# suchapalaver/krust

Measured on AMD Instinct MI355X. Metric: canonical k-mers/s at k=21, 100M x 150bp reads; bit-exact vs krust CPU, higher is better.
Workload: dtype u64; 1 GPU; S100M: 100000000 x 150 bp reads per GPU (rank r: reads [r x 100000000, (r + 1) x 100000000)), k=21, genome 2^27 bp, seed 20260130; resident in HBM; k=21, reads_per_gpu=100000000, distinct_per_gpu=1085824844, table_slots=2147483648, capacity_hint=1115311478, parallelism=reads sharded x1

## Files before the change

krust_amd/csrc/batch.hip:

```cpp
#include "ctx.hip.h"
#include "level1_api.h"

namespace khi {

template <bool QUAL>
void launch_count(kh_ctx *c, const uint8_t *abase, const uint8_t *qbase, int qaligned, u64 vbeg, u64 vend,
                  u64 wlo, u64 tile0, u64 ntiles) {
    u64 blocks = ntiles < (u64)grid_cap() ? ntiles : (u64)grid_cap();
    uint32_t tpb = (uint32_t)((ntiles + blocks - 1) / blocks);
    blocks = (ntiles + tpb - 1) / tpb;
    uint32_t thr = 0;
    if (QUAL) {
        int t = c->minq + 33;
        thr = (uint32_t)(t > 255 ? 255 : t);
    }
    hipLaunchKernelGGL(kh::count_direct_kernel<QUAL>, dim3((unsigned)blocks), dim3(kh::BLOCK), 0, c->stream, abase,
                       qbase, qaligned, vbeg, vend, wlo, tile0, ntiles, tpb, c->k, thr, table_geom(c, c->table, c->cap), c->d_ctr);
}

struct RangeArgs {
    const uint8_t *abase, *qbase;
    int qaligned;
    bool use_qual;
    u64 vbeg, vend, wlo;
    double survive = 1.0;
};

constexpr int KH_RETRY_FULL_SIZE = 1000;
constexpr int KH_RETRY_WIDE = 1001;

u64 sized_for(u64 n, double survive) {
    if (survive >= 1.0) return n;
    const double e = (double)n * (survive * 1.125 + 1.0 / 64) + 65536.0;
    return e >= (double)n ? n : (u64)e;
}

uint32_t qual_thr(const kh_ctx *c) {
    int t = c->minq + 33;
    return (uint32_t)(t > 255 ? 255 : t);
}

template <typename PT>
void launch_region(kh_ctx *c, const kh::PartGeom &g, u64 nregions, u64 hot, const u64 *bend, bool narrow, u64 skip, u64 expect);
bool region_small_groups(const kh_ctx *c, u64 expect, u64 nregions) {
    const int forced = c->knobs.region_nt;
    if (forced) return forced == 512;
    const double keys = c->est_keys ? (double)(c->distinct_known + c->est_keys) : c->hinted ? (double)c->hint_keys : (double)(c->distinct_known + expect);
    return !(keys > 0.6 * (double)c->cap && expect / nregions > 16384);
}
static bool want_heads(const kh_ctx *c) { return c->comm != nullptr || c->exports_seen || c->knobs.heads_always; }
template <>
void launch_region<u64>(kh_ctx *c, const kh::PartGeom &g, u64 nregions, u64 hot, const u64 *bend, bool, u64 skip, u64 expect) {
    const kh::TableGeom tg = table_geom(c, c->table, c->cap);
#define KH_REGION64(FRESH, NT) \
// ... 168 lines not shown
                               (const uint8_t *)c->rfail, c->d_ctr);
            HIP_TRY(c, hipMemsetAsync(&c->d_ctr->part_failed, 0, sizeof(u64), c->stream));
        }
        HIP_TRY(c, hipGetLastError());
        rc = sync_counters(c);
        if (rc != KH_OK) return rc;
    }
    if (c->h_ctr->hot) {
        const u64 nhot = c->h_ctr->hot, hot_total = c->h_ctr->hot_total;
        const bool crowded = nhot > nregions / 64 && (double)(c->distinct_known + hot_total) > LOAD_HARD * (double)c->cap;
        const bool hot_narrow = sizeof(PT) == 4 && c->narrow && !crowded && c->h_ctr->kmers + hot_total < 0xFFFFFFFFull;
        if (c->trace)
            fprintf(stderr, "[kmerhip] %llu hot bucket(s) (more than %llu payloads each, %llu together) counted apart from the region pass%s\n", nhot,
                    hot_cut, hot_total, hot_narrow ? ", into the 8-byte image" : "");
        if (!hot_narrow && (rc = ensure_wide(c)) != KH_OK) return rc;
        if (crowded) {
            u64 newcap = c->cap * 2;
            while ((double)(c->distinct_known + hot_total) > LOAD_TARGET * (double)newcap) newcap *= 2;
            StageTimer t(c, ST_GROW);
            if ((rc = grow_to(c, newcap)) != KH_OK) return rc;
        }
        {
            StageTimer t(c, ST_MISC);
            if (hot_narrow)
                hipLaunchKernelGGL((kh::hot_buckets_kernel<PT, sizeof(PT) == 4>), dim3(kh::HOT_GRID), dim3(kh::BLOCK), 0, c->stream, table_geom(c, c->table, c->cap), g,
                                   (const PT *)bufB, (const u64 *)c->bstart, bend, (const uint32_t *)c->hot_list, nhot, c->d_ctr, c->ntab);
            else
                hipLaunchKernelGGL((kh::hot_buckets_kernel<PT, false>), dim3(kh::HOT_GRID), dim3(kh::BLOCK), 0, c->stream, table_geom(c, c->table, c->cap), g,
                                   (const PT *)bufB, (const u64 *)c->bstart, bend, (const uint32_t *)c->hot_list, nhot, c->d_ctr, (u64 *)nullptr);
            HIP_TRY(c, hipMemsetAsync(&c->d_ctr->hot, 0, 2 * sizeof(u64), c->stream));
        }
        HIP_TRY(c, hipGetLastError());
        c->rheads_valid = false;
        if ((rc = sync_counters(c)) != KH_OK) return rc;
    }
    if ((double)c->distinct_known > LOAD_PART * (double)c->cap) {
        u64 newcap = c->cap * 2;
        while ((double)c->distinct_known > LOAD_TARGET * (double)newcap) newcap *= 2;
        StageTimer t(c, ST_GROW);
        rc = grow_to(c, newcap);
        if (rc != KH_OK) return rc;
    }
    return KH_OK;
}

template <typename PT>
int partition_batch(kh_ctx *c, const RangeArgs &ra, GeomChoice &gc, u64 tile0, u64 ntiles, bool size_from_sample, double range_scale, bool sized_narrow, bool may_narrow) {
    constexpr bool CHUNKED = true;
    kh::PartGeom &g = gc.g;
    const u64 P1 = 1ull << g.p1_bits;
    const u64 n_all = ntiles * kh::PART_TILE;
    const bool estimated = ra.survive < 1.0;
    const u64 n_ub = sized_for(n_all, ra.survive);
    const u64 pool_chunks = (n_ub / kh::CHUNK_PAY) + (n_ub / kh::CHUNK_PAY) / 24 + (u64)PART_G1 * (P1 + kh::POOL_GRAB) + 1024;
    const u64 max_blocks = pool_chunks / kh::CPB + P1 + 1;
    int rc;
    if (!c->moff) {
        u64 z = 0;
        z = 0;
        if ((rc = ensure_buf(c, &c->moff, &z, (u64)kh::MAX_P1 + 1, "hipMalloc(moff)")) != KH_OK) return rc;
        z = 0;
        if ((rc = ensure_buf(c, &c->nch, &z, (u64)kh::MAX_P1 + 1, "hipMalloc(nch)")) != KH_OK) return rc;
        z = 0;
        if ((rc = ensure_buf(c, &c->info, &z, 8, "hipMalloc(info)")) != KH_OK) return rc;
        z = 0;
        if ((rc = ensure_buf(c, &c->pcount, &z, (u64)kh::MAX_P1, "hipMalloc(pcount)")) != KH_OK) return rc;
        z = 0;
        if ((rc = ensure_buf(c, &c->pstart, &z, (u64)kh::MAX_P1 + 1, "hipMalloc(pstart)")) != KH_OK) return rc;
        z = 0;
        if ((rc = ensure_buf(c, &c->pool_next, &z, 1, "hipMalloc(pool_next)")) != KH_OK) return rc;
        z = 0;
        if ((rc = ensure_buf(c, &c->ptotal, &z, (u64)kh::MAX_P1, "hipMalloc(ptotal)")) != KH_OK) return rc;
        z = 0;
        if ((rc = ensure_buf(c, &c->pcap, &z, (u64)kh::MAX_P1, "hipMalloc(pcap)")) != KH_OK) return rc;
        z = 0;
        if ((rc = ensure_buf(c, &c->ovf, &z, 4, "hipMalloc(ovf)")) != KH_OK) return rc;
        z = 0;
        if ((rc = ensure_buf(c, &c->heavy, &z, (u64)kh::MAX_P1, "hipMalloc(heavy)")) != KH_OK) return rc;
    }
    if ((rc = ensure_buf(c, &c->blocks, &c->blocks_cap, max_blocks, "hipMalloc(blocks)")) != KH_OK) return rc;
    if (c->pool_cap < pool_chunks) {
        u64 z = c->chunk_part ? c->pool_cap : 0;
        if ((rc = ensure_buf(c, &c->chunk_part, &z, pool_chunks, "hipMalloc(chunk_part)")) != KH_OK) return rc;
        z = c->fill8 ? c->pool_cap : 0;
        if ((rc = ensure_buf(c, &c->fill8, &z, pool_chunks, "hipMalloc(fill8)")) != KH_OK) return rc;
        z = c->plist ? c->pool_cap : 0;
        if ((rc = ensure_buf(c, &c->plist, &z, pool_chunks, "hipMalloc(plist)")) != KH_OK) return rc;
        c->pool_cap = pool_chunks;
    }
    const u64 a_bytes = pool_chunks * kh::CHUNK_PAY * sizeof(PT);
    if (c->key_cap < a_bytes) {
        u64 z = c->keysA ? c->key_cap : 0;
        if ((rc = ensure_buf(c, &c->keysA, &z, a_bytes, "hipMalloc(keysA)")) != KH_OK) return rc;
        c->key_cap = a_bytes;
    }
    const uint32_t est_np = size_from_sample ? (uint32_t)std::min<u64>(16, std::max<u64>(1, (2ull << 20) / std::max<u64>(1, n_ub / P1))) : 0u;
    constexpr uint32_t EST_P0 = 517;
    u64 est_slots = 0;
    uint32_t est_sub = 0;
    if (size_from_sample) {
        while (est_sub < 6 && (n_ub / P1) >> (est_sub + 1) >= (1ull << 19)) ++est_sub;
        est_slots = 1ull << 16;
        while (est_slots < 3 * (u64)est_np * ((n_ub / P1 >> est_sub) + 1)) est_slots *= 2;
        if ((rc = ensure_buf(c, &c->est_set, &c->est_set_cap, est_slots, "hipMalloc(distinct sample)")) != KH_OK) return rc;
    }

    const uint32_t tpb = (uint32_t)((ntiles + PART_G1 - 1) / PART_G1);
// ... 512 lines not shown
```

krust_amd/csrc/level1.hip.h:

```cpp
#pragma once
#include <utility>

#include "part_common.hip.h"
#include "window.hip.h"

namespace kh {

struct ChunkDst {
    u64 a;
    u64 b;
};
constexpr u64 CHUNK_DST_DROP = 1ull << 63;

template <bool QUAL, int MODE, bool FAST, typename PT, int KT>
__global__ __launch_bounds__(PART_NT) void part1_scatter_chunked_kernel(
    const uint8_t *__restrict__ abase, const uint8_t *__restrict__ qbase, int qaligned, u64 vbeg, u64 vend, u64 wlo,
    u64 tile0, u64 ntiles, uint32_t tiles_per_block, uint32_t k, uint32_t thr, PartGeom g, PT *__restrict__ pool,
    uint16_t *__restrict__ chunk_part, uint8_t *__restrict__ fill8, u64 *__restrict__ pool_next, u64 pool_chunks,
    Counters *ctr) {
    constexpr int ROUNDS = sizeof(PT) == 8 ? 2 : 1;
    constexpr int WPR = CHUNK / ROUNDS;
    constexpr int RTILE = PART_NT * WPR;
    __shared__ uint32_t s_code[2][PART_NT + 2];
    __shared__ uint16_t s_val[2][PART_NT + 2];
    __shared__ PT s_stage[RTILE + 2];
    __shared__ uint16_t s_pid[RTILE + 2];
    __shared__ uint32_t s_cnt[MAX_P1];
    __shared__ uint32_t s_meta[MAX_P1];
    __shared__ ChunkDst s_dst[MAX_P1];
    __shared__ uint32_t s_wsum[4];
    __shared__ uint16_t s_lofs[MAX_P1];
    __shared__ u64 s_priv_next, s_priv_end;
    const int tid = threadIdx.x;
    if (KT) k = KT;
    const uint32_t p1b = (KT == 21 && FAST) ? 10u : g.p1_bits;
    s_cnt[tid] = 0;
    if (tid == 0) {
        s_priv_next = atomicAdd(pool_next, (u64)POOL_GRAB);
        s_priv_end = s_priv_next + POOL_GRAB;
    }
    u64 cur = 0;
    uint32_t fill = CHUNK_PAY;
    bool have_chunk = false;
    const u64 tb = tile0 + (u64)blockIdx.x * tiles_per_block;
    u64 te = tb + tiles_per_block;
    if (te > tile0 + ntiles) te = tile0 + ntiles;
    int buf = 0;
    uint32_t lost = 0;
    __syncthreads();
    {
        const RawChunk raw0 = load_raw<QUAL>(abase, qbase, qaligned, chunk_pos<PART_NT>(tb, tid), vbeg, tb < te ? vend : 0);
        stage_encode<QUAL, PART_NT>(s_code, s_val, 0, true, tid, raw0, abase, qbase, qaligned, tb, vbeg, vend, thr);
    }
    for (u64 t = tb; t < te; ++t, buf ^= 1) {
        __syncthreads();
// ... 87 lines not shown
            __syncthreads();
            s_cnt[tid] = 0;
            if (tid == 0 && s_priv_next + POOL_LOW > s_priv_end) {
                s_priv_next = atomicAdd(pool_next, (u64)POOL_GRAB);
                s_priv_end = s_priv_next + POOL_GRAB;
            }
            if (h == 0)
                stage_encode<QUAL, PART_NT>(s_code, s_val, buf ^ 1, false, tid, raw, abase, qbase, qaligned, t + 1, vbeg, vend, thr);
#if !(KH_ABL & 4)
#pragma unroll 2
            for (uint32_t i = tid; i < total; i += PART_NT) {
                const uint32_t p = s_pid[i];
                const uint32_t meta = s_meta[p];
                const ChunkDst d = s_dst[p];
                const uint32_t e = i - (meta & 0xFFFFu);
#if KH_ABL & 2
                if (s_stage[i] == 0x12345678u && e == 77 && d.a == 5) pool[0] = 1;
#else
                if (e < (meta >> 16)) pool[d.a + i] = s_stage[i];
                else if (d.b != CHUNK_DST_DROP) pool[d.b + i] = s_stage[i];
#endif
            }
#endif
            if (h + 1 < ROUNDS) __syncthreads();
        }
    }
    if (have_chunk) fill8[cur] = (uint8_t)(fill - 1);
    const u64 l = wave_sum((u64)lost);
    if (lane_id() == 0 && l) atomicAdd(&ctr->failed, l);
}

constexpr uint32_t P1B_CAP = 32;
constexpr uint32_t P1B_WORDS = MAX_P1 * P1B_CAP;

__device__ __forceinline__ uint32_t rev2_complement(uint32_t x) {
    const uint32_t y = __builtin_bitreverse32(~x);
    return ((y >> 1) & 0x55555555u) | ((y & 0x55555555u) << 1);
}

typedef __attribute__((address_space(3))) uint32_t lds_u32;
#ifndef KH_L1_SWIZZLE
#define KH_L1_SWIZZLE 1
#endif
constexpr uint32_t L1_ROT_MASK = KH_L1_SWIZZLE ? 0x70u : 0u;
constexpr uint32_t K21_CNT_OFF = 0;
constexpr uint32_t K21_BIN_OFF = (MAX_P1 + PART_NT) * 4;
constexpr uint32_t K21_TRASH_OFF = K21_BIN_OFF + P1B_WORDS * 4;
constexpr uint32_t K21_WASTE0 = 0x10000u;
__device__ __forceinline__ uint32_t l1_bin_offset(uint32_t p) { return (p << 7) | ((p << 4) & L1_ROT_MASK); }
__device__ __forceinline__ uint32_t l1_word(uint32_t p, uint32_t w) { return w ^ (((p << 4) & L1_ROT_MASK) >> 2); }
__device__ __forceinline__ uint32_t l1_word64(uint32_t p, uint32_t w) { return w ^ (((p << 4) & L1_ROT_MASK) >> 3); }
__device__ __forceinline__ uint32_t l1_unit(uint32_t p, uint32_t u) { return u ^ (((p << 4) & L1_ROT_MASK) >> 4); }

template <bool QUAL, int MODE, bool FAST, int KW>
__global__ __launch_bounds__(PART_NT) void part1_bins_kernel(
    const uint8_t *__restrict__ abase, const uint8_t *__restrict__ qbase, int qaligned, u64 vbeg, u64 vend, u64 wlo,
    u64 tile0, u64 ntiles, uint32_t tiles_per_block, uint32_t k_rt, uint32_t thr, PartGeom g, uint32_t *__restrict__ pool,
    uint16_t *__restrict__ chunk_part, uint8_t *__restrict__ fill8, u64 *__restrict__ pool_next, u64 pool_chunks,
    Counters *ctr) {
    constexpr bool ASM = KW != 0;
    const uint32_t k = ASM ? (uint32_t)KW : k_rt, p1b = ASM ? 10u : g.p1_bits;
    constexpr int HALF = CHUNK / 2;
    constexpr uint32_t SEG = 16;
    __shared__ __attribute__((aligned(16))) uint32_t s_mem[(K21_TRASH_OFF + 16) / 4];
    __shared__ uint32_t s_code[2][PART_NT + 2];
    __shared__ uint16_t s_val[2][PART_NT + 2];
    __shared__ uint32_t s_flag;
    __shared__ u64 s_priv_next, s_priv_end;
    uint32_t *const s_cnt = s_mem + K21_CNT_OFF / 4;
    uint32_t *const s_bin = s_mem + K21_BIN_OFF / 4;
    __attribute__((address_space(3))) char *const lds = (__attribute__((address_space(3))) char *)s_mem;
    const int tid = threadIdx.x;
    s_cnt[tid] = 0;
    s_cnt[MAX_P1 + tid] = K21_WASTE0;
    if (tid == 0) {
        s_flag = 0;
        s_priv_next = atomicAdd(pool_next, (u64)POOL_GRAB);
        s_priv_end = s_priv_next + POOL_GRAB;
    }
    u64 cur = 0;
    uint32_t fill = CHUNK_PAY;
    uint32_t res = 0;
    bool have_chunk = false;
    const u64 tb = tile0 + (u64)blockIdx.x * tiles_per_block;
    u64 te = tb + tiles_per_block;
    if (te > tile0 + ntiles) te = tile0 + ntiles;
    int buf = 0;
    uint32_t lost = 0;
    const uint32_t waste = K21_CNT_OFF + 4u * (MAX_P1 + (uint32_t)tid);
    uint32_t *const bin = s_bin + (uint32_t)tid * P1B_CAP;
    __syncthreads();
    auto take_chunk = [&](u64 &first) -> bool {
        first = atomicAdd(&s_priv_next, 1ull);
        if (first + 1 > s_priv_end) first = atomicAdd(pool_next, 1ull);
        if (first + 1 > pool_chunks) return false;
        chunk_part[first] = (uint16_t)tid;
        return true;
    };
    auto flush = [&](uint32_t c) -> uint32_t {
        const uint32_t nseg = c / SEG;
        const uint32_t bseg = min(nseg, P1B_CAP / SEG);
        const uint32_t r = c % SEG;
        uint32_t nout = nseg;
        u64 dst[P1B_CAP / SEG];
        const uint32_t space = (CHUNK_PAY - fill) / SEG;
        u64 ib = 0;
        uint32_t ntaken = 0;
        u64 run_a = cur * CHUNK_PAY + fill, run_b = 0;
        if (nseg > space) {
            const uint32_t need = nseg - space;
            const uint32_t nnew = (need * SEG + CHUNK_PAY - 1) / CHUNK_PAY;
            u64 first = 0;
            bool ok = true;
            if (nnew == 1) ok = take_chunk(first);
            else {
                first = atomicAdd(pool_next, (u64)nnew);
                ok = first + nnew <= pool_chunks;
                if (ok) for (uint32_t q = 0; q < nnew; ++q) chunk_part[first + q] = (uint16_t)tid;
            }
            if (!ok) {
                lost += need * SEG;
                nout = space;
            } else {
                ib = first;
                ntaken = nnew;
                run_b = first * CHUNK_PAY - (u64)space * SEG;
                cur = first + nnew - 1;
                fill = need * SEG - (nnew - 1) * CHUNK_PAY;
                have_chunk = true;
            }
        } else {
            fill += nseg * SEG;
        }
        (void)ib; (void)ntaken;
#pragma unroll
        for (uint32_t sg = 0; sg < P1B_CAP / SEG; ++sg) dst[sg] = (sg < space ? run_a : run_b) + (u64)sg * SEG;
        const uint32_t nb = min(bseg, nout);
        uint4 *const bin4 = reinterpret_cast<uint4 *>(bin);
#pragma unroll
        for (uint32_t sg = 0; sg < P1B_CAP / SEG; ++sg)
            if (sg < nb) {
                uint4 *d = reinterpret_cast<uint4 *>(pool + dst[sg]);
                const uint4 x0 = bin4[l1_unit(tid, 4 * sg)], x1 = bin4[l1_unit(tid, 4 * sg + 1)], x2 = bin4[l1_unit(tid, 4 * sg + 2)],
                            x3 = bin4[l1_unit(tid, 4 * sg + 3)];
                d[0] = x0; d[1] = x1; d[2] = x2; d[3] = x3;
            }
        if (c <= P1B_CAP) {
            if (bseg) {
                const uint32_t nu = (r + 3u) / 4u;
                for (uint32_t i = 0; i < nu; ++i) bin4[l1_unit(tid, i)] = bin4[l1_unit(tid, 4 * bseg + i)];
            }
            s_cnt[tid] = r * 4u;
        } else {
            bin[l1_word(tid, 16)] = (uint32_t)run_a;
            bin[l1_word(tid, 17)] = (uint32_t)(run_a >> 32);
            bin[l1_word(tid, 18)] = (uint32_t)run_b;
            bin[l1_word(tid, 19)] = (uint32_t)(run_b >> 32);
            bin[l1_word(tid, 20)] = space * SEG;
            bin[l1_word(tid, 21)] = nout * SEG;
            bin[l1_word(tid, 22)] = nseg * SEG;
            s_cnt[tid] = (r - (c - P1B_CAP)) * 4u;
        }
        s_cnt[MAX_P1 + tid] = K21_WASTE0;
        return r;
    };
    {
        const RawChunk raw0 = load_raw<QUAL>(abase, qbase, qaligned, chunk_pos<PART_NT>(tb, tid), vbeg, tb < te ? vend : 0);
        stage_encode<QUAL, PART_NT>(s_code, s_val, 0, true, tid, raw0, abase, qbase, qaligned, tb, vbeg, vend, thr);
    }
    for (u64 t = tb; t < te; ++t, buf ^= 1) {
        __syncthreads();
        const RawChunk raw = load_raw<QUAL>(abase, qbase, qaligned, chunk_pos<PART_NT>(t + 1, tid), vbeg, t + 1 < te ? vend : 0);
        const WinCtx w = stage_collect<PART_NT>(s_code, s_val, buf, tid, t);
        const uint32_t good = window_good(w, k, wlo);
        const uint32_t w0 = (uint32_t)w.lo64, w1 = (uint32_t)(w.lo64 >> 32), w2 = w.hi;
        const uint32_t c0 = ASM ? rev2_complement(w2) : 0u, c1 = ASM ? rev2_complement(w1) : 0u, c2 = ASM ? rev2_complement(w0) : 0u;
        Roller roll;
        if (!ASM) roll.init(w, k, wlo);
        auto window = [&](int j, uint32_t &pay, uint32_t &cnta, uint32_t &binb) {
            u64 key;
            const bool ok = roll.next(j, key);
            uint32_t p1 = 0;
            pay = 0;
            if (!QUAL || ok) {
                if (FAST) {
                    hash_p1_pay32<MODE>(k, p1b, key, p1, pay);
                } else {
                    const u64 H = part_hash<MODE>(g, key);
                    pay = Pay<uint32_t>::make(key, H, g);
                    p1 = p1_of_hash(H, g);
                }
            }
            cnta = ok ? K21_CNT_OFF + 4u * p1 : waste;
            binb = l1_bin_offset(p1);
        };
#define KH_W21(J)                                                                                            \
    {                                                                                                        \
        uint32_t cnta;                                                                                       \
        if constexpr (ASM) {                                                                                 \
            uint32_t flo, fhi, rlo, rhi;                                                                     \
            win_fields<KW ? KW : 21, J>(w0, w1, w2, c0, c1, c2, flo, fhi, rlo, rhi);                         \
            win_hash32<KW ? KW : 21, J>(flo, fhi, rlo, rhi, good, waste, L1_ROT_MASK, pay[(J) % HALF], cnta, binb[(J) % HALF]); \
        } else window(J, pay[(J) % HALF], cnta, binb[(J) % HALF]);                                           \
        rk[(J) % HALF] = __hip_atomic_fetch_add((lds_u32 *)(lds + cnta), 4u, __ATOMIC_RELAXED, __HIP_MEMORY_SCOPE_WORKGROUP); \
    }
#pragma unroll
        for (int h = 0; h < 2; ++h) {
            uint32_t omask = 0;
            {
                uint32_t pay[HALF], binb[HALF], rk[HALF];
                if (h == 0) { KH_W21(0) KH_W21(1) KH_W21(2) KH_W21(3) KH_W21(4) KH_W21(5) KH_W21(6) KH_W21(7) }
                else { KH_W21(8) KH_W21(9) KH_W21(10) KH_W21(11) KH_W21(12) KH_W21(13) KH_W21(14) KH_W21(15) }
                uint32_t racc = 0;
#pragma unroll
                for (int j = 0; j < HALF; ++j) {
                    const uint32_t r4 = rk[j];
                    *(lds_u32 *)(lds + K21_BIN_OFF + (r4 < 4u * P1B_CAP ? (binb[j] ^ r4) : K21_TRASH_OFF - K21_BIN_OFF)) = pay[j];
                    racc |= r4;
                }
                if (racc & (K21_WASTE0 - 4u * P1B_CAP)) {
                    s_flag = 1u;
#pragma unroll
                    for (int j = 0; j < HALF; ++j)
                        if (rk[j] >= 4u * P1B_CAP && rk[j] < K21_WASTE0) omask |= 1u << j;
                }
            }
            if (h == 1 && tid == 0 && s_priv_next + 2 * POOL_LOW > s_priv_end) {
                s_priv_next = atomicAdd(pool_next, (u64)POOL_GRAB);
                s_priv_end = s_priv_next + POOL_GRAB;
            }
            __syncthreads();
            const bool slow = s_flag != 0u;
            if (h == 0)
                stage_encode<QUAL, PART_NT>(s_code, s_val, buf ^ 1, false, tid, raw, abase, qbase, qaligned, t + 1, vbeg, vend, thr);
            res = flush(s_cnt[tid] >> 2);
            if (slow) {
                __syncthreads();
                if (omask) {
                    Roller again;
                    again.init(w, k, wlo);
#pragma unroll
                    for (int j = 0; j < CHUNK; ++j) {
                        u64 key;
                        again.next(j, key);
                        if (j / HALF == h && ((omask >> (j % HALF)) & 1u)) {
                            uint32_t p, pv;
                            if (FAST) {
                                hash_p1_pay32<MODE>(k, p1b, key, p, pv);
                            } else {
                                const u64 H = part_hash<MODE>(g, key);
                                pv = Pay<uint32_t>::make(key, H, g);
                                p = p1_of_hash(H, g);
                            }
                            uint32_t *const pbin = s_bin + p * P1B_CAP;
                            const int32_t r2 = (int32_t)atomicAdd(&s_cnt[p], 4u) >> 2;
                            if (r2 >= 0) {
                                pbin[l1_word(p, (uint32_t)r2)] = pv;
                            } else {
                                const u64 ra = ((u64)pbin[l1_word(p, 17)] << 32) | pbin[l1_word(p, 16)];
                                const u64 rb = ((u64)pbin[l1_word(p, 19)] << 32) | pbin[l1_word(p, 18)];
                                const uint32_t split = pbin[l1_word(p, 20)], lim = pbin[l1_word(p, 21)];
                                const uint32_t e = pbin[l1_word(p, 22)] + (uint32_t)r2;
                                if (e < lim) pool[(e < split ? ra : rb) + e] = pv;
                            }
                        }
                    }
                }
                if (tid == 0) s_flag = 0u;
            }
            if (h == 0) __syncthreads();
        }
#undef KH_W21
    }
    __syncthreads();
    res = s_cnt[tid] >> 2;
    if (res) {
        bool room = true;
        if (fill + res > CHUNK_PAY) {
            u64 first;
            room = take_chunk(first);
            if (room) {
                cur = first;
                fill = 0;
                have_chunk = true;
            } else {
                lost += res;
            }
        }
        if (room) {
            for (uint32_t i = 0; i < res; ++i) pool[cur * CHUNK_PAY + fill + i] = bin[l1_word(tid, i)];
            fill += res;
        }
    }
    if (have_chunk) fill8[cur] = (uint8_t)(fill - 1);
    const u64 l = wave_sum((u64)lost);
    if (lane_id() == 0 && l) atomicAdd(&ctr->failed, l);
}

constexpr uint32_t P1B64_CAP = 16;
constexpr uint32_t P1B64_SEG = 8;
constexpr uint32_t K64_BIN_OFF = (MAX_P1 + PART_NT) * 4;
constexpr uint32_t K64_TRASH_OFF = K64_BIN_OFF + MAX_P1 * P1B64_CAP * 8;

template <int... Is, typename F>
__device__ __forceinline__ void static_for_seq(std::integer_sequence<int, Is...>, F &&f) {
    (f(std::integral_constant<int, Is>{}), ...);
}
template <int N, typename F>
__device__ __forceinline__ void static_for(F &&f) {
    static_for_seq(std::make_integer_sequence<int, N>{}, f);
}

template <bool QUAL, int MODE, int KW, int FW>
__global__ __launch_bounds__(PART_NT) void part1_bins64_kernel(
    const uint8_t *__restrict__ abase, const uint8_t *__restrict__ qbase, int qaligned, u64 vbeg, u64 vend, u64 wlo,
    u64 tile0, u64 ntiles, uint32_t tiles_per_block, uint32_t k_rt, uint32_t thr, PartGeom g, u64 *__restrict__ pool,
    uint16_t *__restrict__ chunk_part, uint8_t *__restrict__ fill8, u64 *__restrict__ pool_next, u64 pool_chunks,
    Counters *ctr) {
    constexpr bool ASM = KW != 0;
    const uint32_t k = ASM ? (uint32_t)KW : k_rt;
    constexpr uint32_t SEG = P1B64_SEG, CAP = P1B64_CAP;
    constexpr int NFLUSH = CHUNK / FW;
    __shared__ __attribute__((aligned(16))) uint32_t s_mem[(K64_TRASH_OFF + 16) / 4];
    __shared__ uint32_t s_code[2][PART_NT + 2];
    __shared__ uint16_t s_val[2][PART_NT + 2];
    __shared__ uint32_t s_flag;
    __shared__ u64 s_priv_next, s_priv_end;
    __shared__ uint32_t s_live[QUAL ? 2 : 1][QUAL ? PART_NT : 1];
    __shared__ uint32_t s_nlive[2];
    uint32_t *const s_cnt = s_mem;
    u64 *const s_bin = reinterpret_cast<u64 *>(s_mem + K64_BIN_OFF / 4);
    __attribute__((address_space(3))) char *const lds = (__attribute__((address_space(3))) char *)s_mem;
    typedef __attribute__((address_space(3))) u64 lds_u64;
    const int tid = threadIdx.x;
    s_cnt[tid] = 0;
    s_cnt[MAX_P1 + tid] = K21_WASTE0;
    if (tid == 0) {
        s_flag = 0;
        s_nlive[0] = s_nlive[1] = 0;
        s_priv_next = atomicAdd(pool_next, (u64)POOL_GRAB);
        s_priv_end = s_priv_next + POOL_GRAB;
    }
    u64 cur = 0;
    uint32_t fill = CHUNK_PAY;
    bool have_chunk = false;
    const u64 tb = tile0 + (u64)blockIdx.x * tiles_per_block;
    u64 te = tb + tiles_per_block;
    if (te > tile0 + ntiles) te = tile0 + ntiles;
    int buf = 0;
    uint32_t lost = 0;
    const uint32_t waste = 4u * (MAX_P1 + (uint32_t)tid);
    u64 *const bin = s_bin + (uint32_t)tid * CAP;
    __syncthreads();
    auto take_chunk = [&](u64 &first) -> bool {
        first = atomicAdd(&s_priv_next, 1ull);
        if (first + 1 > s_priv_end) first = atomicAdd(pool_next, 1ull);
        if (first + 1 > pool_chunks) return false;
        chunk_part[first] = (uint16_t)tid;
        return true;
    };
    auto flush = [&](uint32_t c) {
        const uint32_t nseg = c / SEG;
        const uint32_t bseg = min(nseg, CAP / SEG);
        const uint32_t r = c % SEG;
        uint32_t nout = nseg;
        const uint32_t space = (CHUNK_PAY - fill) / SEG;
        u64 run_a = cur * CHUNK_PAY + fill, run_b = 0;
        if (nseg > space) {
            const uint32_t need = nseg - space;
            const uint32_t nnew = (need * SEG + CHUNK_PAY - 1) / CHUNK_PAY;
            u64 first = 0;
            bool ok = true;
            if (nnew == 1) ok = take_chunk(first);
            else {
                first = atomicAdd(pool_next, (u64)nnew);
                ok = first + nnew <= pool_chunks;
                if (ok) for (uint32_t q = 0; q < nnew; ++q) chunk_part[first + q] = (uint16_t)tid;
            }
            if (!ok) {
                lost += need * SEG;
                nout = space;
            } else {
                run_b = first * CHUNK_PAY - (u64)space * SEG;
                cur = first + nnew - 1;
                fill = need * SEG - (nnew - 1) * CHUNK_PAY;
                have_chunk = true;
            }
        } else {
            fill += nseg * SEG;
        }
        const uint32_t nb = min(bseg, nout);
        uint4 *const bin4 = reinterpret_cast<uint4 *>(bin);
#pragma unroll
        for (uint32_t sg = 0; sg < CAP / SEG; ++sg)
            if (sg < nb) {
                uint4 *d = reinterpret_cast<uint4 *>(pool + (sg < space ? run_a : run_b) + (u64)sg * SEG);
                const uint4 x0 = bin4[l1_unit(tid, 4 * sg)], x1 = bin4[l1_unit(tid, 4 * sg + 1)], x2 = bin4[l1_unit(tid, 4 * sg + 2)],
                            x3 = bin4[l1_unit(tid, 4 * sg + 3)];
                d[0] = x0; d[1] = x1; d[2] = x2; d[3] = x3;
            }
        if (c <= CAP) {
            if (bseg) {
                const uint32_t nu = (r + 1u) / 2u;
                for (uint32_t i = 0; i < nu; ++i) bin4[l1_unit(tid, i)] = bin4[l1_unit(tid, 4 * bseg + i)];
            }
            s_cnt[tid] = r * 8u;
        } else {
            bin[l1_word64(tid, 8)] = run_a;
            bin[l1_word64(tid, 9)] = run_b;
            bin[l1_word64(tid, 10)] = (u64)(space * SEG) | ((u64)(nout * SEG) << 32);
            bin[l1_word64(tid, 11)] = (u64)(nseg * SEG);
            s_cnt[tid] = (r - (c - CAP)) * 8u;
        }
        s_cnt[MAX_P1 + tid] = K21_WASTE0;
    };
    auto p1_pay_of = [&](u64 key, u64 &pay) -> uint32_t {
        const u64 H = kh_table_hash<MODE>(key, k) << g.shard_shift;
        pay = H << g.p1_bits;
        return p1_of_hash(H, g);
    };
    {
        const RawChunk raw0 = load_raw<QUAL>(abase, qbase, qaligned, chunk_pos<PART_NT>(tb, tid), vbeg, tb < te ? vend : 0);
        stage_encode<QUAL, PART_NT>(s_code, s_val, 0, true, tid, raw0, abase, qbase, qaligned, tb, vbeg, vend, thr);
    }
#ifndef KH_L1_LIVE_LIST
#define KH_L1_LIVE_LIST 1
#endif
    constexpr bool LIVE = QUAL && KH_L1_LIVE_LIST != 0;
    auto build_list = [&](int cbuf, u64 tt, int lb) {
        WinCtx wn;
        wn.hi = s_code[cbuf][tid];
        wn.lo64 = ((u64)s_code[cbuf][tid + 1] << 32) | s_code[cbuf][tid + 2];
        wn.V = ((u64)s_val[cbuf][tid] << 32) | ((u64)s_val[cbuf][tid + 1] << 16) | (u64)s_val[cbuf][tid + 2];
        wn.p0 = (u64)chunk_pos<PART_NT>(tt, tid);
        const uint32_t gd = window_good(wn, k, wlo);
        const bool live = gd != 0u;
        const u64 m = kh_ballot(live);
        uint32_t lbase = 0;
        if (m) {
            if ((int)lane_id() == __builtin_ctzll(m)) lbase = atomicAdd(&s_nlive[lb], (uint32_t)__builtin_popcountll(m));
            lbase = (uint32_t)__shfl((int)lbase, __builtin_ctzll(m), 64);
        }
        if (live) s_live[lb][lbase + mbcnt(m)] = (uint32_t)tid | (gd << 16);
    };
    if constexpr (LIVE) {
        __syncthreads();
        build_list(0, tb, 0);
    }
    for (u64 t = tb; t < te; ++t, buf ^= 1) {
        __syncthreads();
        const RawChunk raw = load_raw<QUAL>(abase, qbase, qaligned, chunk_pos<PART_NT>(t + 1, tid), vbeg, t + 1 < te ? vend : 0);
        WinCtx w = stage_collect<PART_NT>(s_code, s_val, buf, tid, t);
        uint32_t good = LIVE ? 0u : window_good(w, k, wlo);
        bool wave_busy = true;
        const int lcur = (int)((t - tb) & 1);
        if constexpr (LIVE) {
            const uint32_t nlive = s_nlive[lcur];
            if (tid == 0) s_nlive[lcur ^ 1] = 0;
#ifndef KH_L1_WAVE_ORDER
#define KH_L1_WAVE_ORDER 0
#endif
            const uint32_t wv = (uint32_t)tid >> 6, seg = KH_L1_WAVE_ORDER ? ((wv & 3u) << 2) | (wv >> 2) : wv;
            const uint32_t li = (seg << 6) | ((uint32_t)tid & 63u);
            wave_busy = (seg << 6) < nlive;
            const uint32_t item = li < nlive ? s_live[lcur][li] : 0u;
            const uint32_t c = item & 0xFFFFu;
            good = item >> 16;
            w.hi = s_code[buf][c];
// ... 13 lines not shown
            uint32_t omask = 0;
            if (wave_busy) {
                uint32_t klo[FW], khi[FW], binb[FW], rk[FW];
                static_for<FW>([&](auto jc) {
                    constexpr int j = decltype(jc)::value, J = h * FW + j;
                    uint32_t cnta;
#ifndef KH_L1_WAVE_SKIP
#define KH_L1_WAVE_SKIP 0
#endif
                    if constexpr (ASM) {
                        if (KH_L1_WAVE_SKIP && QUAL && !kh_any(((good >> (15 - J)) & 1u) != 0u)) {
                            klo[j] = khi[j] = 0u;
                            cnta = waste;
                            binb[j] = 0u;
                        } else {
                            uint32_t flo, fhi, rlo, rhi;
                            win_fields<KW ? KW : 31, J>(w0, w1, w2, c0, c1, c2, flo, fhi, rlo, rhi);
                            win_hash64<KW ? KW : 31, J>(flo, fhi, rlo, rhi, good, waste, L1_ROT_MASK, klo[j], khi[j], cnta, binb[j]);
                        }
                    } else {
                        u64 key, pv = 0;
                        const bool ok = roll.next(J, key);
                        uint32_t p = 0;
                        if (!QUAL || ok) p = p1_pay_of(key, pv);
                        klo[j] = (uint32_t)pv;
                        khi[j] = (uint32_t)(pv >> 32);
                        cnta = ok ? 4u * p : waste;
                        binb[j] = l1_bin_offset(p);
                    }
                    rk[j] = __hip_atomic_fetch_add((lds_u32 *)(lds + cnta), 8u, __ATOMIC_RELAXED, __HIP_MEMORY_SCOPE_WORKGROUP);
                });
                uint32_t racc = 0;
#pragma unroll
                for (int j = 0; j < FW; ++j) {
                    const uint32_t r8 = rk[j];
                    *(lds_u64 *)(lds + (r8 < 8u * CAP ? K64_BIN_OFF + (binb[j] ^ r8) : K64_TRASH_OFF)) = ((u64)khi[j] << 32) | klo[j];
                    racc |= r8;
                }
                if (racc & (K21_WASTE0 - 8u * CAP)) {
                    s_flag = 1u;
#pragma unroll
                    for (int j = 0; j < FW; ++j)
                        if (rk[j] >= 8u * CAP && rk[j] < K21_WASTE0) omask |= 1u << j;
                }
            }
            if (h == NFLUSH - 1 && tid == 0 && s_priv_next + 2 * POOL_LOW > s_priv_end) {
                s_priv_next = atomicAdd(pool_next, (u64)POOL_GRAB);
                s_priv_end = s_priv_next + POOL_GRAB;
            }
            __syncthreads();
            const bool slow = s_flag != 0u;
            if (h == 0)
                stage_encode<QUAL, PART_NT>(s_code, s_val, buf ^ 1, false, tid, raw, abase, qbase, qaligned, t + 1, vbeg, vend, thr);
            flush(s_cnt[tid] >> 3);
            if (slow) {
                __syncthreads();
                if (omask) {
                    Roller again;
                    again.init(w, k, wlo);
#pragma unroll
                    for (int j = 0; j < CHUNK; ++j) {
                        u64 key;
                        again.next(j, key);
                        if (j / FW == h && ((omask >> (j % FW)) & 1u)) {
                            u64 pv;
                            const uint32_t p = p1_pay_of(key, pv);
                            u64 *const pbin = s_bin + p * CAP;
                            const int32_t r2 = (int32_t)atomicAdd(&s_cnt[p], 8u) >> 3;
                            if (r2 >= 0) {
                                pbin[l1_word64(p, (uint32_t)r2)] = pv;
                            } else {
                                const u64 ra = pbin[l1_word64(p, 8)], rb = pbin[l1_word64(p, 9)];
                                const u64 d10 = pbin[l1_word64(p, 10)];
                                const uint32_t split = (uint32_t)d10, lim = (uint32_t)(d10 >> 32);
                                const uint32_t e = (uint32_t)pbin[l1_word64(p, 11)] + (uint32_t)r2;
                                if (e < lim) pool[(e < split ? ra : rb) + e] = pv;
                            }
                        }
                    }
                }
                if (tid == 0) s_flag = 0u;
            }
            if (h + 1 < NFLUSH) __syncthreads();
            if constexpr (LIVE && h == 0 && NFLUSH > 1) build_list(buf ^ 1, t + 1, lcur ^ 1);
        });
        if constexpr (LIVE && NFLUSH == 1) {
            __syncthreads();
            build_list(buf ^ 1, t + 1, lcur ^ 1);
        }
    }
    __syncthreads();
    const uint32_t res = s_cnt[tid] >> 3;
    if (res) {
        bool room = true;
        if (fill + res > CHUNK_PAY) {
            u64 first;
            room = take_chunk(first);
            if (room) {
                cur = first;
                fill = 0;
                have_chunk = true;
            } else {
                lost += res;
            }
        }
        if (room) {
            for (uint32_t i = 0; i < res; ++i) pool[cur * CHUNK_PAY + fill + i] = bin[l1_word64(tid, i)];
            fill += res;
        }
    }
    if (have_chunk) fill8[cur] = (uint8_t)(fill - 1);
    const u64 l = wave_sum((u64)lost);
    if (lane_id() == 0 && l) atomicAdd(&ctr->failed, l);
}

}
```

Before: 206.0 billion k-mers/s.

## Allocate pool chunks in multi-chunk runs and rework L1 bin flush addressing

New measurement: 209.4 billion k-mers/s (median of 3 runs). About the same (+1.6%).

```diff
diff --git a/krust_amd/csrc/batch.hip b/krust_amd/csrc/batch.hip
--- a/krust_amd/csrc/batch.hip
+++ b/krust_amd/csrc/batch.hip
@@ -1,5 +1,6 @@
 #include "ctx.hip.h"
 #include "level1_api.h"
+#include "l1_flush_bits.h"
 
 namespace khi {
 
@@ -274,7 +275,8 @@
     const u64 n_all = ntiles * kh::PART_TILE;
     const bool estimated = ra.survive < 1.0;
     const u64 n_ub = sized_for(n_all, ra.survive);
-    const u64 pool_chunks = (n_ub / kh::CHUNK_PAY) + (n_ub / kh::CHUNK_PAY) / 24 + (u64)PART_G1 * (P1 + kh::POOL_GRAB) + 1024;
+    const u64 pool_chunks = (n_ub / kh::CHUNK_PAY) + (n_ub / kh::CHUNK_PAY) / 24 + (u64)PART_G1 * (P1 + kh::POOL_GRAB) + 1024 +
+                            kh::l1f_idle_tail_chunks((u64)PART_G1, P1);
     const u64 max_blocks = pool_chunks / kh::CPB + P1 + 1;
     int rc;
     if (!c->moff) {
diff --git a/krust_amd/csrc/l1_flush_bits.h b/krust_amd/csrc/l1_flush_bits.h
--- /dev/null
+++ b/krust_amd/csrc/l1_flush_bits.h
@@ -0,0 +1,54 @@
+#pragma once
+#include <stdint.h>
+
+#if defined(__HIPCC__)
+#define KH_HD __host__ __device__ __forceinline__
+#else
+#define KH_HD inline
+#endif
+
+namespace kh {
+
+constexpr uint32_t L1F_UNIT = 16;
+constexpr uint32_t L1F_SEG = 64;
+constexpr uint32_t L1F_BIN = 128;
+#ifndef KH_L1F_RUN
+#define KH_L1F_RUN 4
+#endif
+constexpr uint32_t L1F_RUN = KH_L1F_RUN;
+
+KH_HD constexpr uint32_t l1f_held(uint32_t cb) { return cb < L1F_BIN ? cb : L1F_BIN; }
+KH_HD constexpr uint32_t l1f_bin_segs(uint32_t cb) { return l1f_held(cb) / L1F_SEG; }
+KH_HD constexpr uint32_t l1f_run_segs(uint32_t cb) { return cb / L1F_SEG; }
+KH_HD constexpr uint32_t l1f_first_unit(uint32_t cb) { return (l1f_held(cb) & ~(L1F_UNIT - 1u)) - l1f_bin_segs(cb) * L1F_SEG; }
+KH_HD constexpr uint32_t l1f_seg_unit(uint32_t u0, uint32_t i) { return (i * L1F_UNIT) ^ (i * L1F_UNIT < u0 ? L1F_SEG : 0u); }
+KH_HD constexpr bool l1f_moves(uint32_t cb) { return l1f_bin_segs(cb) == 1u && (cb & (L1F_UNIT - 1u)) != 0u; }
+KH_HD constexpr uint32_t l1f_move_src(uint32_t u0) { return u0 + L1F_SEG; }
+KH_HD constexpr uint32_t l1f_left(uint32_t cb) { return cb <= L1F_BIN ? (cb & (L1F_SEG - 1u)) : (cb & (L1F_SEG - 1u)) - (cb - L1F_BIN); }
+KH_HD constexpr uint32_t l1f_unit_addr(uint32_t rot_bin, uint32_t unit_off) { return rot_bin ^ unit_off; }
+
+KH_HD constexpr uint32_t l1f_run_bytes(uint32_t chunk_bytes) { return L1F_RUN * chunk_bytes; }
+KH_HD constexpr uint32_t l1f_beyond(uint32_t fill, uint32_t need, uint32_t chunk_bytes) {
+    return fill + need > l1f_run_bytes(chunk_bytes) ? fill + need - l1f_run_bytes(chunk_bytes) : 0u;
+}
+KH_HD constexpr uint32_t l1f_runs_for(uint32_t beyond, uint32_t chunk_bytes) {
+    return (beyond + l1f_run_bytes(chunk_bytes) - 1u) / l1f_run_bytes(chunk_bytes);
+}
+KH_HD constexpr uint32_t l1f_fill_after(uint32_t beyond, uint32_t chunk_bytes) {
+    return beyond - (l1f_runs_for(beyond, chunk_bytes) - 1u) * l1f_run_bytes(chunk_bytes);
+}
+template <typename A>
+KH_HD constexpr A l1f_run_b(A fresh, uint32_t space) { return fresh - space; }
+template <typename A>
+KH_HD constexpr A l1f_dst(A run_a, A run_b, uint32_t space, uint32_t e) { return (e < space ? run_a : run_b) + e; }
+template <typename A>
+KH_HD constexpr A l1f_run_after(A fresh, uint32_t beyond, uint32_t chunk_bytes) {
+    return fresh + (uint64_t)(l1f_runs_for(beyond, chunk_bytes) - 1u) * l1f_run_bytes(chunk_bytes);
+}
+KH_HD constexpr uint32_t l1f_last_chunk(uint32_t fill, uint32_t chunk_bytes) { return (fill - 1u) / chunk_bytes; }
+KH_HD constexpr uint32_t l1f_last_fill8(uint32_t fill, uint32_t chunk_bytes, uint32_t pay_bytes) {
+    return (fill - l1f_last_chunk(fill, chunk_bytes) * chunk_bytes) / pay_bytes - 1u;
+}
+KH_HD constexpr uint64_t l1f_idle_tail_chunks(uint64_t workgroups, uint64_t partitions) { return workgroups * partitions * (L1F_RUN - 1u); }
+
+}
diff --git a/krust_amd/csrc/level1.hip.h b/krust_amd/csrc/level1.hip.h
--- a/krust_amd/csrc/level1.hip.h
+++ b/krust_amd/csrc/level1.hip.h
@@ -1,6 +1,7 @@
 #pragma once
 #include <utility>
 
+#include "l1_flush_bits.h"
 #include "part_common.hip.h"
 #include "window.hip.h"
 
@@ -194,6 +195,153 @@
 __device__ __forceinline__ uint32_t l1_word64(uint32_t p, uint32_t w) { return w ^ (((p << 4) & L1_ROT_MASK) >> 3); }
 __device__ __forceinline__ uint32_t l1_unit(uint32_t p, uint32_t u) { return u ^ (((p << 4) & L1_ROT_MASK) >> 4); }
 
+struct L1Own {
+    char *run;
+    uint32_t fill;
+    uint32_t lost;
+};
+typedef __attribute__((address_space(3))) char lds_char;
+typedef uint32_t l1_v4u __attribute__((ext_vector_type(4)));
+typedef __attribute__((address_space(3))) l1_v4u lds_u128;
+
+__device__ __forceinline__ bool l1_take_chunks(uint32_t tid, uint32_t n, bool priv, u64 *s_priv_next, const u64 *s_priv_end,
+                                               u64 *__restrict__ pool_next, u64 pool_chunks, uint16_t *__restrict__ chunk_part,
+                                               u64 &first) {
+    first = priv ? atomicAdd(s_priv_next, (u64)n) : ~0ull;
+    if (!priv || first + n > *s_priv_end) first = atomicAdd(pool_next, (u64)n);
+    if (first + n > pool_chunks) return false;
+    for (uint32_t q = 0; q < n; ++q) chunk_part[first + q] = (uint16_t)tid;
+    return true;
+}
+
+template <typename PT>
+__device__ __forceinline__ void l1_flush(lds_char *lds, uint32_t bins, uint32_t tid, L1Own &o, PT *__restrict__ pool,
+                                         uint16_t *__restrict__ chunk_part, u64 *__restrict__ pool_next, u64 pool_chunks,
+                                         u64 *s_priv_next, const u64 *s_priv_end) {
+    constexpr uint32_t CB = CHUNK_PAY * (uint32_t)sizeof(PT), RB = l1f_run_bytes(CB);
+    lds_u32 *const cnt = (lds_u32 *)(lds + 4u * tid);
+#if KH_ABL & 32
+    *cnt = 0u;
+    *(lds_u32 *)(lds + 4u * (MAX_P1 + tid)) = K21_WASTE0;
+    return;
+#endif
+    const uint32_t cb = *cnt;
+    const uint32_t rot = bins + l1_bin_offset(tid);
+    const uint32_t u0 = l1f_first_unit(cb);
+    uint32_t nb = l1f_bin_segs(cb);
+    l1_v4u x0, x1, x2, x3, y0, y1, y2, y3;
+    if (nb >= 1u) {
+        x0 = *(lds_u128 *)(lds + l1f_unit_addr(rot, l1f_seg_unit(u0, 0)));
+        x1 = *(lds_u128 *)(lds + l1f_unit_addr(rot, l1f_seg_unit(u0, 1)));
+        x2 = *(lds_u128 *)(lds + l1f_unit_addr(rot, l1f_seg_unit(u0, 2)));
+        x3 = *(lds_u128 *)(lds + l1f_unit_addr(rot, l1f_seg_unit(u0, 3)));
+    }
+    if (nb == 2u) {
+        y0 = *(lds_u128 *)(lds + l1f_unit_addr(rot, L1F_SEG));
+        y1 = *(lds_u128 *)(lds + l1f_unit_addr(rot, L1F_SEG + L1F_UNIT));
+        y2 = *(lds_u128 *)(lds + l1f_unit_addr(rot, L1F_SEG + 2u * L1F_UNIT));
+        y3 = *(lds_u128 *)(lds + l1f_unit_addr(rot, L1F_SEG + 3u * L1F_UNIT));
+    }
+    if (l1f_moves(cb)) {
+        const l1_v4u m = *(lds_u128 *)(lds + l1f_unit_addr(rot, l1f_move_src(u0)));
+        *(lds_u128 *)(lds + l1f_unit_addr(rot, u0)) = m;
+    }
+    const uint32_t need = l1f_run_segs(cb) * L1F_SEG;
+    char *d0 = o.run + o.fill, *d1 = d0 + L1F_SEG;
+    if (__builtin_expect(cb > L1F_BIN || o.fill + need > RB, 0)) {
+        const uint32_t space = RB - o.fill;
+        const uint32_t beyond = l1f_beyond(o.fill, need, CB);
+        char *const run_a = d0;
+        char *run_b = d0;
+        uint32_t nout = need;
+        if (beyond) {
+            const uint32_t nrun = l1f_runs_for(beyond, CB);
+            u64 first;
+            if (l1_take_chunks(tid, nrun * L1F_RUN, nrun == 1u, s_priv_next, s_priv_end, pool_next, pool_chunks, chunk_part, first)) {
+                char *const fresh = reinterpret_cast<char *>(pool) + first * CB;
+                run_b = l1f_run_b(fresh, space);
+                o.run = l1f_run_after(fresh, beyond, CB);
+                o.fill = l1f_fill_after(beyond, CB);
+            } else {
+                o.lost += beyond / (uint32_t)sizeof(PT);
+                nout = space;
+                o.fill = RB;
+            }
+        } else {
+            o.fill += need;
+        }
+        d0 = l1f_dst(run_a, run_b, space, 0u);
+        d1 = l1f_dst(run_a, run_b, space, L1F_SEG);
+        nb = min(nb, nout / L1F_SEG);
+        if (cb > L1F_BIN) {
+            const char *const p0 = reinterpret_cast<const char *>(pool);
+            const u64 ia = (u64)((int64_t)(run_a - p0) / (int64_t)sizeof(PT)), ib = (u64)((int64_t)(run_b - p0) / (int64_t)sizeof(PT));
+            const uint32_t split = space / (uint32_t)sizeof(PT);
+            const uint32_t lim = nout / (uint32_t)sizeof(PT);
+            const uint32_t end = need / (uint32_t)sizeof(PT);
+            if constexpr (sizeof(PT) == 4) {
+                *(lds_u32 *)(lds + (rot ^ 64u)) = (uint32_t)ia;
+                *(lds_u32 *)(lds + (rot ^ 68u)) = (uint32_t)(ia >> 32);
+                *(lds_u32 *)(lds + (rot ^ 72u)) = (uint32_t)ib;
+                *(lds_u32 *)(lds + (rot ^ 76u)) = (uint32_t)(ib >> 32);
+                *(lds_u32 *)(lds + (rot ^ 80u)) = split;
+                *(lds_u32 *)(lds + (rot ^ 84u)) = lim;
+                *(lds_u32 *)(lds + (rot ^ 88u)) = end;
+            } else {
+                typedef __attribute__((address_space(3))) u64 lds_u64;
+                *(lds_u64 *)(lds + (rot ^ 64u)) = ia;
+                *(lds_u64 *)(lds + (rot ^ 72u)) = ib;
+                *(lds_u64 *)(lds + (rot ^ 80u)) = (u64)split | ((u64)lim << 32);
+                *(lds_u64 *)(lds + (rot ^ 88u)) = (u64)end;
+            }
+        }
+    } else {
+        o.fill += need;
+    }
+    if (nb >= 1u) {
+        l1_v4u *const d = reinterpret_cast<l1_v4u *>(d0);
+        d[0] = x0; d[1] = x1; d[2] = x2; d[3] = x3;
+    }
+    if (nb == 2u) {
+        l1_v4u *const d = reinterpret_cast<l1_v4u *>(d1);
+        d[0] = y0; d[1] = y1; d[2] = y2; d[3] = y3;
+    }
+    *cnt = l1f_left(cb);
+    *(lds_u32 *)(lds + 4u * (MAX_P1 + tid)) = K21_WASTE0;
+}
+
+template <typename PT>
+__device__ __forceinline__ void l1_finish(lds_char *lds, uint32_t bins, uint32_t tid, L1Own &o, PT *__restrict__ pool,
+                                          uint16_t *__restrict__ chunk_part, uint8_t *__restrict__ fill8, u64 *__restrict__ pool_next,
+                                          u64 pool_chunks, u64 *s_priv_next, const u64 *s_priv_end, Counters *ctr) {
+    constexpr uint32_t CB = CHUNK_PAY * (uint32_t)sizeof(PT), RB = l1f_run_bytes(CB);
+    typedef __attribute__((address_space(3))) PT lds_pay;
+    const uint32_t rb = *(lds_u32 *)(lds + 4u * tid);
+    const uint32_t rot = bins + l1_bin_offset(tid);
+    if (rb && o.fill == RB) {
+        u64 first;
+        if (l1_take_chunks(tid, 1u, true, s_priv_next, s_priv_end, pool_next, pool_chunks, chunk_part, first)) {
+            PT *const d = reinterpret_cast<PT *>(reinterpret_cast<char *>(pool) + first * CB);
+            for (uint32_t b = 0; b < rb; b += (uint32_t)sizeof(PT)) d[b / sizeof(PT)] = *(lds_pay *)(lds + (rot ^ b));
+            fill8[first] = (uint8_t)(rb / (uint32_t)sizeof(PT) - 1u);
+        } else {
+            o.lost += rb / (uint32_t)sizeof(PT);
+        }
+    } else if (rb) {
+        PT *const d = reinterpret_cast<PT *>(o.run + o.fill);
+        for (uint32_t b = 0; b < rb; b += (uint32_t)sizeof(PT)) d[b / sizeof(PT)] = *(lds_pay *)(lds + (rot ^ b));
+        o.fill += rb;
+    }
+    if (o.fill != RB) {
+        const u64 c0 = (u64)(o.run - reinterpret_cast<char *>(pool)) / CB;
+        const uint32_t last = l1f_last_chunk(o.fill, CB);
+        fill8[c0 + last] = (uint8_t)l1f_last_fill8(o.fill, CB, (uint32_t)sizeof(PT));
+        for (uint32_t q = last + 1u; q < L1F_RUN; ++q) chunk_part[c0 + q] = PART_NONE;
+    }
+    const u64 l = wave_sum((u64)o.lost);
+    if (lane_id() == 0 && l) atomicAdd(&ctr->failed, l);
+}
+
 template <bool QUAL, int MODE, bool FAST, int KW>
 __global__ __launch_bounds__(PART_NT) void part1_bins_kernel(
     const uint8_t *__restrict__ abase, const uint8_t *__restrict__ qbase, int qaligned, u64 vbeg, u64 vend, u64 wlo,
@@ -203,7 +351,6 @@
     constexpr bool ASM = KW != 0;
     const uint32_t k = ASM ? (uint32_t)KW : k_rt, p1b = ASM ? 10u : g.p1_bits;
     constexpr int HALF = CHUNK / 2;
-    constexpr uint32_t SEG = 16;
     __shared__ __attribute__((aligned(16))) uint32_t s_mem[(K21_TRASH_OFF + 16) / 4];
     __shared__ uint32_t s_code[2][PART_NT + 2];
     __shared__ uint16_t s_val[2][PART_NT + 2];
@@ -220,92 +367,16 @@
         s_priv_next = atomicAdd(pool_next, (u64)POOL_GRAB);
         s_priv_end = s_priv_next + POOL_GRAB;
     }
-    u64 cur = 0;
-    uint32_t fill = CHUNK_PAY;
-    uint32_t res = 0;
-    bool have_chunk = false;
+    L1Own own;
+    own.run = reinterpret_cast<char *>(pool);
+    own.fill = l1f_run_bytes(CHUNK_PAY * 4u);
+    own.lost = 0;
     const u64 tb = tile0 + (u64)blockIdx.x * tiles_per_block;
     u64 te = tb + tiles_per_block;
     if (te > tile0 + ntiles) te = tile0 + ntiles;
     int buf = 0;
-    uint32_t lost = 0;
     const uint32_t waste = K21_CNT_OFF + 4u * (MAX_P1 + (uint32_t)tid);
-    uint32_t *const bin = s_bin + (uint32_t)tid * P1B_CAP;
     __syncthreads();
-    auto take_chunk = [&](u64 &first) -> bool {
-        first = atomicAdd(&s_priv_next, 1ull);
-        if (first + 1 > s_priv_end) first = atomicAdd(pool_next, 1ull);
-        if (first + 1 > pool_chunks) return false;
-        chunk_part[first] = (uint16_t)tid;
-        return true;
-    };
-    auto flush = [&](uint32_t c) -> uint32_t {
-        const uint32_t nseg = c / SEG;
-        const uint32_t bseg = min(nseg, P1B_CAP / SEG);
-        const uint32_t r = c % SEG;
-        uint32_t nout = nseg;
-        u64 dst[P1B_CAP / SEG];
-        const uint32_t space = (CHUNK_PAY - fill) / SEG;
-        u64 ib = 0;
-        uint32_t ntaken = 0;
-        u64 run_a = cur * CHUNK_PAY + fill, run_b = 0;
-        if (nseg > space) {
-            const uint32_t need = nseg - space;
-            const uint32_t nnew = (need * SEG + CHUNK_PAY - 1) / CHUNK_PAY;
-            u64 first = 0;
-            bool ok = true;
-            if (nnew == 1) ok = take_chunk(first);
-            else {
-                first = atomicAdd(pool_next, (u64)nnew);
-                ok = first + nnew <= pool_chunks;
-                if (ok) for (uint32_t q = 0; q < nnew; ++q) chunk_part[first + q] = (uint16_t)tid;
-            }
-            if (!ok) {
-                lost += need * SEG;
-                nout = space;
-            } else {
-                ib = first;
-                ntaken = nnew;
-                run_b = first * CHUNK_PAY - (u64)space * SEG;
-                cur = first + nnew - 1;
-                fill = need * SEG - (nnew - 1) * CHUNK_PAY;
-                have_chunk = true;
-            }
-        } else {
-            fill += nseg * SEG;
-        }
-        (void)ib; (void)ntaken;
-#pragma unroll
-        for (uint32_t sg = 0; sg < P1B_CAP / SEG; ++sg) dst[sg] = (sg < space ? run_a : run_b) + (u64)sg * SEG;
-        const uint32_t nb = min(bseg, nout);
-        uint4 *const bin4 = reinterpret_cast<uint4 *>(bin);
-#pragma unroll
-        for (uint32_t sg = 0; sg < P1B_CAP / SEG; ++sg)
-            if (sg < nb) {
-                uint4 *d = reinterpret_cast<uint4 *>(pool + dst[sg]);
-                const uint4 x0 = bin4[l1_unit(tid, 4 * sg)], x1 = bin4[l1_unit(tid, 4 * sg + 1)], x2 = bin4[l1_unit(tid, 4 * sg + 2)],
-                            x3 = bin4[l1_unit(tid, 4 * sg + 3)];
-                d[0] = x0; d[1] = x1; d[2] = x2; d[3] = x3;
-            }
-        if (c <= P1B_CAP) {
-            if (bseg) {
-                const uint32_t nu = (r + 3u) / 4u;
-                for (uint32_t i = 0; i < nu; ++i) bin4[l1_unit(tid, i)] = bin4[l1_unit(tid, 4 * bseg + i)];
-            }
-            s_cnt[tid] = r * 4u;
-        } else {
-            bin[l1_word(tid, 16)] = (uint32_t)run_a;
-            bin[l1_word(tid, 17)] = (uint32_t)(run_a >> 32);
-            bin[l1_word(tid, 18)] = (uint32_t)run_b;
-            bin[l1_word(tid, 19)] = (uint32_t)(run_b >> 32);
-            bin[l1_word(tid, 20)] = space * SEG;
-            bin[l1_word(tid, 21)] = nout * SEG;
-            bin[l1_word(tid, 22)] = nseg * SEG;
-            s_cnt[tid] = (r - (c - P1B_CAP)) * 4u;
-        }
-        s_cnt[MAX_P1 + tid] = K21_WASTE0;
-        return r;
-    };
     {
         const RawChunk raw0 = load_raw<QUAL>(abase, qbase, qaligned, chunk_pos<PART_NT>(tb, tid), vbeg, tb < te ? vend : 0);
         stage_encode<QUAL, PART_NT>(s_code, s_val, 0, true, tid, raw0, abase, qbase, qaligned, tb, vbeg, vend, thr);
@@ -375,7 +446,7 @@
             const bool slow = s_flag != 0u;
             if (h == 0)
                 stage_encode<QUAL, PART_NT>(s_code, s_val, buf ^ 1, false, tid, raw, abase, qbase, qaligned, t + 1, vbeg, vend, thr);
-            res = flush(s_cnt[tid] >> 2);
+            l1_flush<uint32_t>(lds, K21_BIN_OFF, (uint32_t)tid, own, pool, chunk_part, pool_next, pool_chunks, &s_priv_next, &s_priv_end);
             if (slow) {
                 __syncthreads();
                 if (omask) {
@@ -415,28 +486,7 @@
 #undef KH_W21
     }
     __syncthreads();
-    res = s_cnt[tid] >> 2;
-    if (res) {
-        bool room = true;
-        if (fill + res > CHUNK_PAY) {
-            u64 first;
-            room = take_chunk(first);
-            if (room) {
-                cur = first;
-                fill = 0;
-                have_chunk = true;
-            } else {
-                lost += res;
-            }
-        }
-        if (room) {
-            for (uint32_t i = 0; i < res; ++i) pool[cur * CHUNK_PAY + fill + i] = bin[l1_word(tid, i)];
-            fill += res;
-        }
-    }
-    if (have_chunk) fill8[cur] = (uint8_t)(fill - 1);
-    const u64 l = wave_sum((u64)lost);
-    if (lane_id() == 0 && l) atomicAdd(&ctr->failed, l);
+    l1_finish<uint32_t>(lds, K21_BIN_OFF, (uint32_t)tid, own, pool, chunk_part, fill8, pool_next, pool_chunks, &s_priv_next, &s_priv_end, ctr);
 }
 
 constexpr uint32_t P1B64_CAP = 16;
@@ -461,7 +511,7 @@
     Counters *ctr) {
     constexpr bool ASM = KW != 0;
     const uint32_t k = ASM ? (uint32_t)KW : k_rt;
-    constexpr uint32_t SEG = P1B64_SEG, CAP = P1B64_CAP;
+    constexpr uint32_t CAP = P1B64_CAP;
     constexpr int NFLUSH = CHUNK / FW;
     __shared__ __attribute__((aligned(16))) uint32_t s_mem[(K64_TRASH_OFF + 16) / 4];
     __shared__ uint32_t s_code[2][PART_NT + 2];
@@ -483,79 +533,16 @@
         s_priv_next = atomicAdd(pool_next, (u64)POOL_GRAB);
         s_priv_end = s_priv_next + POOL_GRAB;
     }
-    u64 cur = 0;
-    uint32_t fill = CHUNK_PAY;
-    bool have_chunk = false;
+    L1Own own;
+    own.run = reinterpret_cast<char *>(pool);
+    own.fill = l1f_run_bytes(CHUNK_PAY * 8u);
+    own.lost = 0;
     const u64 tb = tile0 + (u64)blockIdx.x * tiles_per_block;
     u64 te = tb + tiles_per_block;
     if (te > tile0 + ntiles) te = tile0 + ntiles;
     int buf = 0;
-    uint32_t lost = 0;
     const uint32_t waste = 4u * (MAX_P1 + (uint32_t)tid);
-    u64 *const bin = s_bin + (uint32_t)tid * CAP;
     __syncthreads();
-    auto take_chunk = [&](u64 &first) -> bool {
-        first = atomicAdd(&s_priv_next, 1ull);
-        if (first + 1 > s_priv_end) first = atomicAdd(pool_next, 1ull);
-        if (first + 1 > pool_chunks) return false;
-        chunk_part[first] = (uint16_t)tid;
-        return true;
-    };
-    auto flush = [&](uint32_t c) {
-        const uint32_t nseg = c / SEG;
-        const uint32_t bseg = min(nseg, CAP / SEG);
-        const uint32_t r = c % SEG;
-        uint32_t nout = nseg;
-        const uint32_t space = (CHUNK_PAY - fill) / SEG;
-        u64 run_a = cur * CHUNK_PAY + fill, run_b = 0;
-        if (nseg > space) {
-            const uint32_t need = nseg - space;
-            const uint32_t nnew = (need * SEG + CHUNK_PAY - 1) / CHUNK_PAY;
-            u64 first = 0;
-            bool ok = true;
-            if (nnew == 1) ok = take_chunk(first);
-            else {
-                first = atomicAdd(pool_next, (u64)nnew);
-                ok = first + nnew <= pool_chunks;
-                if (ok) for (uint32_t q = 0; q < nnew; ++q) chunk_part[first + q] = (uint16_t)tid;
-            }
-            if (!ok) {
-                lost += need * SEG;
-                nout = space;
-            } else {
-                run_b = first * CHUNK_PAY - (u64)space * SEG;
-                cur = first + nnew - 1;
-                fill = need * SEG - (nnew - 1) * CHUNK_PAY;
-                have_chunk = true;
-            }
-        } else {
-            fill += nseg * SEG;
-        }
-        const uint32_t nb = min(bseg, nout);
-        uint4 *const bin4 = reinterpret_cast<uint4 *>(bin);
-#pragma unroll
-        for (uint32_t sg = 0; sg < CAP / SEG; ++sg)
-            if (sg < nb) {
-                uint4 *d = reinterpret_cast<uint4 *>(pool + (sg < space ? run_a : run_b) + (u64)sg * SEG);
-                const uint4 x0 = bin4[l1_unit(tid, 4 * sg)], x1 = bin4[l1_unit(tid, 4 * sg + 1)], x2 = bin4[l1_unit(tid, 4 * sg + 2)],
-                            x3 = bin4[l1_unit(tid, 4 * sg + 3)];
-                d[0] = x0; d[1] = x1; d[2] = x2; d[3] = x3;
-            }
-        if (c <= CAP) {
-            if (bseg) {
-                const uint32_t nu = (r + 1u) / 2u;
-                for (uint32_t i = 0; i < nu; ++i) bin4[l1_unit(tid, i)] = bin4[l1_unit(tid, 4 * bseg + i)];
-            }
-            s_cnt[tid] = r * 8u;
-        } else {
-            bin[l1_word64(tid, 8)] = run_a;
-            bin[l1_word64(tid, 9)] = run_b;
-            bin[l1_word64(tid, 10)] = (u64)(space * SEG) | ((u64)(nout * SEG) << 32);
-            bin[l1_word64(tid, 11)] = (u64)(nseg * SEG);
-            s_cnt[tid] = (r - (c - CAP)) * 8u;
-        }
-        s_cnt[MAX_P1 + tid] = K21_WASTE0;
-    };
     auto p1_pay_of = [&](u64 key, u64 &pay) -> uint32_t {
         const u64 H = kh_table_hash<MODE>(key, k) << g.shard_shift;
         pay = H << g.p1_bits;
@@ -675,7 +662,7 @@
             const bool slow = s_flag != 0u;
             if (h == 0)
                 stage_encode<QUAL, PART_NT>(s_code, s_val, buf ^ 1, false, tid, raw, abase, qbase, qaligned, t + 1, vbeg, vend, thr);
-            flush(s_cnt[tid] >> 3);
+            l1_flush<u64>(lds, K64_BIN_OFF, (uint32_t)tid, own, pool, chunk_part, pool_next, pool_chunks, &s_priv_next, &s_priv_end);
             if (slow) {
                 __syncthreads();
                 if (omask) {
@@ -713,28 +700,7 @@
         }
     }
     __syncthreads();
-    const uint32_t res = s_cnt[tid] >> 3;
-    if (res) {
-        bool room = true;
-        if (fill + res > CHUNK_PAY) {
-            u64 first;
-            room = take_chunk(first);
-            if (room) {
-                cur = first;
-                fill = 0;
-                have_chunk = true;
-            } else {
-                lost += res;
-            }
-        }
-        if (room) {
-            for (uint32_t i = 0; i < res; ++i) pool[cur * CHUNK_PAY + fill + i] = bin[l1_word64(tid, i)];
-            fill += res;
-        }
-    }
-    if (have_chunk) fill8[cur] = (uint8_t)(fill - 1);
-    const u64 l = wave_sum((u64)lost);
-    if (lane_id() == 0 && l) atomicAdd(&ctr->failed, l);
-}
-
-}
+    l1_finish<u64>(lds, K64_BIN_OFF, (uint32_t)tid, own, pool, chunk_part, fill8, pool_next, pool_chunks, &s_priv_next, &s_priv_end, ctr);
+}
+
+}
```
